# WeijingShi/Point-GNN

Measured on AMD Instinct MI355X. Metric: KITTI-shaped frames/sec (car_auto_T3 inference: graph build + GNN, 20000 pts/frame, mean E1 602k), higher is better.
Workload: dtype f32

## Files before the change

### include/pointgnn_hip.h

```cpp
#ifndef POINTGNN_HIP_H_
#define POINTGNN_HIP_H_

#include <stddef.h>
#include <stdint.h>

#ifdef __cplusplus
extern "C" {
#endif

#define PGNN_E_INVALID (-1)
#define PGNN_E_WORKSPACE (-2)
#define PGNN_E_UNSUPPORTED (-3)
#define PGNN_E_CAPACITY (-4)
#define PGNN_E_COMM (-5)

int pgnn_version(void);
const char *pgnn_last_error(void);
int pgnn_check_device_pointer(const void *device_ptr);

int pgnn_stream_create_cu_mask(int32_t cu_first, int32_t cu_count,
                               int32_t complement, void **stream_out);
int pgnn_stream_destroy(void *stream);

int pgnn_scatter_max_f32(const float *data, int64_t ld_data,
// ... 951 lines not shown
                     const uint8_t *scales, int32_t scale,
                     const uint8_t *colors, int64_t n_colors,
                     const uint8_t *plate_colors, int64_t n_plate_colors,
                     void *workspace, size_t workspace_bytes, void *stream);
int pgnn_render_font(uint8_t *table_host );

size_t pgnn_png_unfilter_workspace_bytes(int64_t width, int64_t height);
int pgnn_png_unfilter(const uint8_t *raw, int64_t width, int64_t height,
                      int32_t color_type, const uint8_t *palette,
                      int32_t palette_entries, int32_t bgr, void *workspace,
                      size_t workspace_bytes, uint8_t *image, void *stream);

size_t pgnn_png_encode_workspace_bytes(int64_t height, int64_t width,
                                       int32_t chunk_bytes);
int pgnn_png_encode(const uint8_t *image, int64_t height, int64_t width,
                    int64_t row_stride_bytes, int32_t chunk_bytes,
                    void *workspace, size_t workspace_bytes, uint8_t *out,
                    int64_t out_capacity, int64_t *out_bytes_dev, void *stream);

int pgnn_set_tunable(const char *key, int value);
int pgnn_kernel_occupancy(const char *kernel, int64_t lds_bytes,
                          int32_t *vgprs, int32_t *scratch_bytes,
                          int32_t *workgroups_per_cu, int64_t *lds_used);
int pgnn_set_debug_buffer(void *device_ptr);

#ifdef __cplusplus
}
#endif
#endif
```

### point-gnn_amd/_lib.py

```python
import ctypes
import os

import torch

from . import _header

_HERE = os.path.dirname(os.path.abspath(__file__))
LIB_PATH = os.environ.get("PGNN_LIB") or os.path.join(_HERE, "libpointgnn_hip.so")

c_i32, c_i64, c_vp = ctypes.c_int32, ctypes.c_int64, ctypes.c_void_p

_S, _C = _header.structs(), _header.constants()

FcLayer = _S["pgnn_fc_layer"]
DynCount = _S["pgnn_dyn_count"]
WgradJob = _S["pgnn_wgrad_job"]
MergeJob = _S["pgnn_merge_job"]
FrameArrays = _S["pgnn_frame_arrays"]
TrainFc = _S["pgnn_train_fc"]
TrainStage = _S["pgnn_train_stage"]
TrainModel = _S["pgnn_train_model"]
TrainBatch = _S["pgnn_train_batch"]


# ... 113 lines not shown
        return ctypes.byref(DynCount(self.dev.data_ptr(), self.hint))


def tag_count(t, count):
    if count is not None:
        t._pgnn_count = count
    return t


def count_of(t):
    return getattr(t, "_pgnn_count", None) if t is not None else None


def kernel_occupancy(kernel, lds_bytes=-1):
    v, sc, wg = c_i32(0), c_i32(0), c_i32(0)
    used = c_i64(0)
    check(load().pgnn_kernel_occupancy(
        kernel.encode(), int(lds_bytes), ctypes.byref(v), ctypes.byref(sc),
        ctypes.byref(wg), ctypes.byref(used)), "pgnn_kernel_occupancy")
    return {"vgprs": v.value, "scratch_bytes": sc.value,
            "workgroups_per_cu": wg.value, "lds_bytes": used.value}


def set_tunable(key, value):
    check(load().pgnn_set_tunable(key.encode(), int(value)), "pgnn_set_tunable")
```

### point-gnn_amd/csrc/gnn.hip

```cpp
#include <atomic>

#include "mlp_engine.h"
#include "edge_ws.h"
#include "edge_ws_split.h"
#include "pool_ws.h"
#include "pool_split.h"
#include "pool_ws_f16.h"

namespace pgnn {
int g_mlp_blocks_per_cu = 4;
int g_edge_msub = 0;
int g_pool_msub = 0;
int g_mlp_pool_pct = 12;
int g_ws_xcds = 8;
int g_ws_prio = 1;
int g_f16_pool = 1;
int g_b16_force = 0;
int g_ws_pool_pct = 0;
int g_ws_chunk = 2;
int g_ws_balance = 1;
int g_ws_reserve = 0;
void *g_mlp_ts = nullptr;
int g_mlp_debug = 0;
}
// ... 2366 lines not shown
      PGNN_REQUIRE(lds_bytes >= 0 && lds_bytes <= 160 * 1024, PGNN_E_INVALID,
                   "kernel_occupancy: no launch of this kernel yet, or more "
                   "LDS than a CU has");
      if (lds_bytes) {
        const int rc = ensure_dynamic_lds(table[i].fn[dyn], (size_t)lds_bytes);
        if (rc) return rc;
      }
      hipFuncAttributes attr;
      PGNN_HIP(hipFuncGetAttributes(&attr, table[i].fn[dyn]));
      int blocks = 0;
      PGNN_HIP(hipOccupancyMaxActiveBlocksPerMultiprocessor(
          &blocks, table[i].fn[dyn], 64 * kRowsWaves, (size_t)lds_bytes));
      *vgprs = attr.numRegs;
      *scratch_bytes = (int32_t)attr.localSizeBytes;
      *workgroups_per_cu = blocks;
      if (lds_used) *lds_used = lds_bytes;
      return 0;
    }
  PGNN_REQUIRE(false, PGNN_E_INVALID, "kernel_occupancy: unknown kernel");
  return 0;
  PGNN_GUARD_END
}

extern "C" int pgnn_point_set_pooling_rows_fwd(
    const float *point_features, int32_t n_feat, const float *point_xyz,
    const int32_t *keypoint_indices, const int32_t *edges, int64_t n_edges,
    int32_t num_keypoints, const pgnn_fc_layer *layers, int32_t n_layers,
    int32_t edges_sorted, float *out, int64_t ld_out, float *const *acts_host,
    int64_t ld_last, void *stream_) {
  PGNN_GUARD_BEGIN
  hipStream_t stream = (hipStream_t)stream_;
  PGNN_REQUIRE(n_edges >= 0 && num_keypoints >= 0 && n_feat >= 0 && n_feat <= 13 &&
                   layers && acts_host,
               PGNN_E_INVALID, "point_set_pooling_rows: bad sizes");
  if (n_layers != 4) return PGNN_E_UNSUPPORTED;
  Plan p;
  int rc = make_plan(layers, n_layers, n_feat + 3, p);
  if (rc) return rc;
  const int out_cols = 16 * p.chain.l[n_layers - 1].nt;
  PGNN_REQUIRE(out && ld_out >= out_cols && ld_last >= out_cols && ld_last % 4 == 0,
               PGNN_E_INVALID, "point_set_pooling_rows: bad output");
  const int cus = ws_cus(stream);
  if (n_edges == 0 || num_keypoints == 0 || !pool_ws_applies(p, n_edges, cus))
    return PGNN_E_UNSUPPORTED;
  PGNN_REQUIRE(point_xyz && keypoint_indices && edges && (n_feat == 0 || point_features),
               PGNN_E_INVALID, "point_set_pooling_rows: null input");
// ... 73 lines not shown
```

### point-gnn_amd/csrc/graph.hip

```cpp
#include <math.h>

#include <mutex>
#include <vector>

#include "kdtree.h"
#include "npy_divmod.h"
#include "sort.h"

namespace pgnn {
namespace {

struct __attribute__((aligned(32))) SortedPoint {
  double x, y, z;
  int32_t idx;
  int32_t pad;
};

__device__ __forceinline__ uint32_t cell_hash(int cx, int cy, int cz,
                                              uint32_t mask) {
  uint32_t h = (uint32_t)cx * 73856093u ^ (uint32_t)cy * 19349663u ^
               (uint32_t)cz * 83492791u;
  h ^= h >> 15;
  return h & mask;
}
// ... 82 lines not shown
                                   int32_t *__restrict__ vcell_sorted,
                                   const int32_t *__restrict__ n_dev) {
  graph_prio();
  if (n_dev) n = *n_dev < n ? *n_dev : n;
  for (int64_t i = (int64_t)blockIdx.x * blockDim.x + threadIdx.x; i < n;
       i += (int64_t)gridDim.x * blockDim.x) {
    const uint32_t k = keys[i];
    if (i == 0 || keys[i - 1] != k) cell_start[k] = (int32_t)i;
    if (i == n - 1 || keys[i + 1] != k) cell_end[k] = (int32_t)(i + 1);
    SortedPoint sp;
    const uint32_t idx = vals[i];
    load_point(pts, idx, sc, sp.x, sp.y, sp.z);
    sp.idx = (int32_t)idx;
    sp.pad = 0;
    sorted[i] = sp;
    if (vcell) {
      vcell_sorted[3 * i] = vcell[3 * (int64_t)idx];
      vcell_sorted[3 * i + 1] = vcell[3 * (int64_t)idx + 1];
      vcell_sorted[3 * i + 2] = vcell[3 * (int64_t)idx + 2];
    }
  }
}

template <bool FILL, typename T>
__global__ __launch_bounds__(1024) void radius_query_kernel(
    const T *__restrict__ centers, int64_t n_centers, Scale3 sc, double r,
    uint32_t mask, const int32_t *__restrict__ cell_start,
    const int32_t *__restrict__ cell_end,
    const SortedPoint *__restrict__ sorted, int32_t *__restrict__ counts,
    const int32_t *__restrict__ offsets, int32_t *__restrict__ edges,
    int64_t capacity, const int32_t *__restrict__ n_centers_dev) {
  graph_prio();
  const int lane = threadIdx.x & 63;
  const int wpb = blockDim.x >> 6;
  const int64_t wave0 = (int64_t)blockIdx.x * wpb + (threadIdx.x >> 6);
  const int64_t n_waves = (int64_t)gridDim.x * wpb;
  const int64_t cap = n_centers;
  if (n_centers_dev)
    n_centers = *n_centers_dev < cap ? *n_centers_dev : cap;
  const double r2 = r * r;
  const double inv_r = 1.0 / r;
  const double rr = r * (1.0 + 1e-9) + 1e-300;
  for (int64_t q = wave0; q < cap; q += n_waves) {
    if (q >= n_centers) {
      if (!FILL && lane == 0) counts[q] = 0;
      continue;
    }
    double cx, cy, cz;
    load_point(centers, q, sc, cx, cy, cz);
    const int x0 = rcell_of(cx - rr, inv_r), x1 = rcell_of(cx + rr, inv_r);
    const int y0 = rcell_of(cy - rr, inv_r), y1 = rcell_of(cy + rr, inv_r);
    const int z0 = rcell_of(cz - rr, inv_r), z1 = rcell_of(cz + rr, inv_r);
    const int nx = x1 - x0 + 1, ny = y1 - y0 + 1, nz = z1 - z0 + 1;
    const int n_cells = nx * ny * nz;
    int my_s = 0, my_cnt = 0, my_ix = 0, my_iy = 0, my_iz = 0;
    if (lane < n_cells) {
      my_ix = x0 + lane % nx;
      my_iy = y0 + (lane / nx) % ny;
      my_iz = z0 + lane / (nx * ny);
      const uint32_t b = cell_hash(my_ix, my_iy, my_iz, mask);
      my_s = cell_start[b];
      my_cnt = cell_end[b] - my_s;
    }
    int incl = my_cnt;
#pragma unroll
    for (int d = 1; d < 64; d <<= 1) {
      const int t = __shfl_up(incl, d);
      if (lane >= d) incl += t;
    }
    const int total_cand = __shfl(incl, 63);
    int64_t out_pos = FILL ? (int64_t)offsets[q] : 0;
    int total = 0;
    for (int j0 = 0; j0 < total_cand; j0 += 128) {
      const bool two = j0 + 64 < total_cand;
      bool valid[2];
      int ix[2], iy[2], iz[2];
      SortedPoint sp[2];
#pragma unroll
      for (int u = 0; u < 2; ++u) {
        if (u == 1 && !two) break;
        valid[u] = j0 + 64 * u + lane < total_cand;
        const int j = valid[u] ? j0 + 64 * u + lane : total_cand - 1;
        int lo = 0, hi = n_cells - 1;
#pragma unroll
        for (int step = 0; step < 6; ++step) {
          const int mid = (lo + hi) >> 1;
          const int v = __shfl(incl, mid);
          if (v > j) hi = mid; else lo = mid + 1;
        }
        const int c = lo < n_cells ? lo : n_cells - 1;
        const int c_incl = __shfl(incl, c), c_cnt = __shfl(my_cnt, c);
        const int c_s = __shfl(my_s, c);
        ix[u] = __shfl(my_ix, c);
// ... 337 lines not shown
  if ((threadIdx.x & 63) == 0) {
    atomicMin(&ordered_min[0], m0);
    atomicMin(&ordered_min[1], m1);
    atomicMin(&ordered_min[2], m2);
  }
}

__global__ void grid_origin_kernel(
    const unsigned long long *__restrict__ ordered_min, double sub_x,
    double sub_y, double sub_z, int mode, double *__restrict__ origin) {
  graph_prio();
  if (threadIdx.x == 0 && blockIdx.x == 0) {
    const double sub[3] = {sub_x, sub_y, sub_z};
    for (int ax = 0; ax < 3; ++ax) {
      const double mn = ordered_to_double(ordered_min[ax]);
      origin[ax] = mn - sub[ax];
      origin[3 + ax] = sub[ax];
      origin[6 + ax] = mn;
    }
    origin[9] = (double)mode;
  }
}

__global__ void voxel_leader_kernel(const SortedPoint *__restrict__ sorted,
                                    const uint32_t *__restrict__ keys, int64_t n,
                                    const int32_t *__restrict__ vc,
                                    const int32_t *__restrict__ cell_start,
                                    const int32_t *__restrict__ cell_end,
                                    int32_t *__restrict__ is_leader,
                                    double *__restrict__ centroid,
                                    int32_t *__restrict__ member_count) {
  graph_prio();
  for (int64_t i = (int64_t)blockIdx.x * blockDim.x + threadIdx.x; i < n;
       i += (int64_t)gridDim.x * blockDim.x) {
    const int vx = vc[3 * i], vy = vc[3 * i + 1], vz = vc[3 * i + 2];
    const uint32_t b = keys[i];
    const int s = cell_start[b], e = cell_end[b];
    bool leader;
    if (vc[3 * s] == vx && vc[3 * s + 1] == vy && vc[3 * s + 2] == vz) {
      leader = (int)i == s;
    } else {
      leader = true;
      for (int j = s; j < (int)i; ++j) {
        if (vc[3 * j] == vx && vc[3 * j + 1] == vy && vc[3 * j + 2] == vz) {
          leader = false;
          break;
        }
      }
    }
    is_leader[i] = leader ? 1 : 0;
    if (!leader) continue;
    double sx = 0.0, sy = 0.0, sz = 0.0;
    int cnt = 0;
    int j = (int)i;
    for (; j + 4 <= e; j += 4) {
      int ax[4], ay[4], az[4];
      SortedPoint o[4];
#pragma unroll
      for (int u = 0; u < 4; ++u) {
        ax[u] = vc[3 * (j + u)];
        ay[u] = vc[3 * (j + u) + 1];
        az[u] = vc[3 * (j + u) + 2];
        o[u] = sorted[j + u];
      }
#pragma unroll
      for (int u = 0; u < 4; ++u) {
        const bool m = ax[u] == vx && ay[u] == vy && az[u] == vz;
        sx = m ? sx + o[u].x : sx;
        sy = m ? sy + o[u].y : sy;
        sz = m ? sz + o[u].z : sz;
        cnt += m ? 1 : 0;
      }
    }
    for (; j < e; ++j) {
      const int ax = vc[3 * j], ay = vc[3 * j + 1], az = vc[3 * j + 2];
      const SortedPoint o = sorted[j];
      const bool m = ax == vx && ay == vy && az == vz;
      sx = m ? sx + o.x : sx;
      sy = m ? sy + o.y : sy;
      sz = m ? sz + o.z : sz;
      cnt += m ? 1 : 0;
    }
    centroid[3 * i] = sx / (double)cnt;
    centroid[3 * i + 1] = sy / (double)cnt;
    centroid[3 * i + 2] = sz / (double)cnt;
    member_count[i] = cnt;
  }
}

__global__ __launch_bounds__(1024) void voxel_nn_kernel(
    const SortedPoint *__restrict__ sorted, int64_t n,
    const double *__restrict__ origin, double voxel, uint32_t mask,
    const int32_t *__restrict__ cell_start, const int32_t *__restrict__ cell_end,
    const int32_t *__restrict__ is_leader, const int32_t *__restrict__ slot,
    const double *__restrict__ centroid, const float *__restrict__ pts,
    KdView kd, int32_t *__restrict__ kp_idx, float *__restrict__ kp_xyz,
    int spw ) {
  graph_prio();
  const int lane = threadIdx.x & 63;
  const int wpb = blockDim.x >> 6;
  const int64_t n_waves = (int64_t)gridDim.x * wpb;
  const double ox = origin[0], oy = origin[1], oz = origin[2];
  for (int64_t base = ((int64_t)blockIdx.x * wpb + (threadIdx.x >> 6)) * spw;
       base < n; base += n_waves * spw) {
    unsigned long long leaders = __ballot(
        lane < spw && base + lane < n && is_leader[base + lane] != 0);
    while (leaders) {
      const int64_t i = base + __builtin_ctzll(leaders);
      leaders &= leaders - 1;
      const double cx = centroid[3 * i], cy = centroid[3 * i + 1],
                   cz = centroid[3 * i + 2];
      const int vx = cell_of(cx, ox, voxel), vy = cell_of(cy, oy, voxel),
                vz = cell_of(cz, oz, voxel);
      int my_s = 0, my_cnt = 0, my_ix = 0, my_iy = 0, my_iz = 0;
      if (lane < 27) {
        my_ix = vx - 1 + lane % 3;
        my_iy = vy - 1 + (lane / 3) % 3;
        my_iz = vz - 1 + lane / 9;
        const uint32_t b = cell_hash(my_ix, my_iy, my_iz, mask);
        my_s = cell_start[b];
        my_cnt = cell_end[b] - my_s;
      }
      int incl = my_cnt;
#pragma unroll
      for (int d = 1; d < 32; d <<= 1) {
        const int t = __shfl_up(incl, d);
        if (lane >= d) incl += t;
      }
      const int total_cand = __shfl(incl, 26);
      double best = 1.0e300;
      int best_idx = 0x7fffffff;
      for (int j0 = 0; j0 < total_cand; j0 += 64) {
        const bool valid = j0 + lane < total_cand;
        const int j = valid ? j0 + lane : total_cand - 1;
        int lo = 0, hi = 26;
#pragma unroll
        for (int step = 0; step < 5; ++step) {
          const int mid = (lo + hi) >> 1;
          const int v = __shfl(incl, mid);
          if (v > j) hi = mid; else lo = mid + 1;
        }
        const int c = lo < 27 ? lo : 26;
        const int c_incl = __shfl(incl, c), c_cnt = __shfl(my_cnt, c);
        const int c_s = __shfl(my_s, c);
        const int ix = __shfl(my_ix, c), iy = __shfl(my_iy, c),
                  iz = __shfl(my_iz, c);
        if (valid) {
          const SortedPoint o = sorted[c_s + (j - (c_incl - c_cnt))];
          if (cell_of(o.x, ox, voxel) == ix && cell_of(o.y, oy, voxel) == iy &&
              cell_of(o.z, oz, voxel) == iz) {
            const double ex = o.x - cx, ey = o.y - cy, ez = o.z - cz;
            const double d2 = (ex * ex + ey * ey) + ez * ez;
// ... 1247 lines not shown
extern "C" int pgnn_voxel_keypoints_random(
    const float *points, int64_t n_points, double voxel_size,
    const double *jitter3_host, uint64_t seed, void *workspace,
    size_t workspace_bytes, int32_t *keypoint_indices, float *keypoint_xyz,
    int32_t *num_keypoints, void *stream) {
  PGNN_GUARD_BEGIN
  return keypoints_impl(points, n_points, voxel_size, false, jitter3_host, seed,
                        workspace, workspace_bytes, keypoint_indices,
                        keypoint_xyz, num_keypoints, (hipStream_t)stream);
  PGNN_GUARD_END
}

extern "C" int pgnn_voxel_keypoints_random_f64(
    const double *points, int64_t n_points, double voxel_size,
    const double *jitter3_host, uint64_t seed, void *workspace,
    size_t workspace_bytes, int32_t *keypoint_indices, double *keypoint_xyz,
    int32_t *num_keypoints, void *stream) {
  PGNN_GUARD_BEGIN
  return keypoints_impl(points, n_points, voxel_size, false, jitter3_host, seed,
                        workspace, workspace_bytes, keypoint_indices,
                        keypoint_xyz, num_keypoints, (hipStream_t)stream);
  PGNN_GUARD_END
}
```

### point-gnn_amd/csrc/kdtree.hip

```cpp
#include "kdtree.h"
#include "pgnn_common.h"

namespace pgnn {
namespace {

struct __attribute__((aligned(16))) Rec {
  float c[3];
  int32_t idx;
};
typedef float kd_v4 __attribute__((ext_vector_type(4)));

#ifndef PGNN_KD_NT
#define PGNN_KD_NT 1024
#endif
#ifndef PGNN_KD_LDS_CAP
#define PGNN_KD_LDS_CAP 5120
#endif
#ifndef PGNN_KD_BATCH
#define PGNN_KD_BATCH 2048
#endif
constexpr int KD_NT = PGNN_KD_NT;
constexpr int KD_NW = KD_NT / 64;
constexpr int KD_LDS_CAP = PGNN_KD_LDS_CAP;
constexpr int KD_BATCH = PGNN_KD_BATCH;
// ... 619 lines not shown
        reinterpret_cast<const void *>(kd_subtree_kernel),
        hipFuncAttributeMaxDynamicSharedMemorySize, (int)dyn));
    attr_set = true;
  }
  hipLaunchKernelGGL(kd_init_kernel, dim3(graph_grid((n + 255) / 256)), dim3(256),
                     graph_lds_pad(), stream, pts, (int)n, rec, kd.status);
  int level0 = 0;
  while (level0 < kd.n_levels - 1 &&
         ((n + ((int64_t)1 << level0) - 1) >> level0) > KD_TOP_LEN) {
    hipLaunchKernelGGL(kd_top_kernel, dim3(graph_grid(1 << level0)), dim3(KD_NT), dyn,
                       stream, rec, (int)n, level0, kd.n_nodes, kd.bounds,
                       kd.status);
    ++level0;
  }
  PGNN_REQUIRE(((n + ((int64_t)1 << level0) - 1) >> level0) <= KD_LDS_CAP,
               PGNN_E_INVALID, "kdtree: leaf larger than the LDS capacity");
  hipLaunchKernelGGL(kd_subtree_kernel, dim3(graph_grid(1 << level0)), dim3(KD_NT), dyn,
                     stream, rec, (int)n, level0, kd.n_levels, kd.n_nodes,
                     kd.bounds, kd.idx, kd.pos, kd.status);
  PGNN_HIP(hipGetLastError());
  return 0;
}

}

using namespace pgnn;

extern "C" int pgnn_kdtree_shape(int64_t n_points, int32_t *n_levels,
                                 int32_t *n_nodes) {
  PGNN_GUARD_BEGIN
  PGNN_REQUIRE(n_points >= 0 && n_levels && n_nodes, PGNN_E_INVALID,
               "kdtree_shape: bad argument");
  int lv, nodes;
  kd_shape(n_points, &lv, &nodes);
  *n_levels = lv;
  *n_nodes = nodes;
  return 0;
  PGNN_GUARD_END
}

extern "C" size_t pgnn_kdtree_workspace_bytes(int64_t n_points) {
  if (n_points < 0) return 0;
  return kd_workspace_bytes(n_points);
}

extern "C" int pgnn_kdtree_replica(const float *points, int64_t n_points,
// ... 26 lines not shown
```

### point-gnn_amd/csrc/pgnn_common.h

```cpp
#pragma once
#include <hip/hip_runtime.h>
#include <stdint.h>
#include <stdio.h>

#include <exception>
#include <string>

#include "pointgnn_hip.h"

namespace pgnn {

std::string &last_error();

inline int fail(int code, const char *msg) {
  last_error() = msg;
  return code;
}

#define PGNN_HIP(expr)                                                        \
  do {                                                                        \
    hipError_t e_ = (expr);                                                   \
    if (e_ != hipSuccess) {                                                   \
      char buf_[256];                                                         \
      snprintf(buf_, sizeof buf_, "%s failed: %s (%s:%d)", #expr,             \
// ... 46 lines not shown
                           __ATOMIC_RELAXED, __HIP_MEMORY_SCOPE_AGENT);
  }
}

#ifndef PGNN_GRAPH_PRIO
#define PGNN_GRAPH_PRIO 0
#endif
__device__ __forceinline__ void graph_prio() {
#if PGNN_GRAPH_PRIO > 0
  __builtin_amdgcn_s_setprio(PGNN_GRAPH_PRIO);
#endif
}

extern int g_graph_lds_pad;
inline size_t graph_lds_pad() { return (size_t)g_graph_lds_pad; }
extern int g_graph_max_wgs;
inline unsigned graph_grid(int64_t natural) {
  if (natural < 1) natural = 1;
  if (g_graph_max_wgs > 0 && natural > g_graph_max_wgs) natural = g_graph_max_wgs;
  return (unsigned)natural;
}
inline unsigned graph_wide_block() { return g_graph_max_wgs > 0 ? 1024u : 256u; }

int device_cu_count();
int stream_cu_count(hipStream_t stream);
int ensure_dynamic_lds(const void *kernel, size_t bytes);
size_t device_max_lds();
int arm_sched(int32_t *sched, hipStream_t stream);

int scatter_sum_strided(const float *data, int64_t ld_data,
                        const int32_t *seg_ids, int64_t seg_stride,
                        int64_t n_rows, int32_t n_cols, int32_t num_segments,
                        float *out, int64_t ld_out, int32_t mean,
                        int32_t *counts_ws, int32_t ids_sorted,
                        hipStream_t stream);
int segment_counts(const int32_t *seg_ids, int64_t seg_stride, int64_t n_rows,
                   const int32_t *n_dev, int32_t num_segments, int32_t *counts,
                   hipStream_t stream);
int segment_mean_finish(float *out, int64_t ld_out, int32_t n_cols,
                        int32_t num_segments, const int32_t *counts,
                        const int32_t *ns_dev, hipStream_t stream);
int mlp_rows_gated(const float *x, int64_t ld_x, int32_t nx, int64_t n_rows,
                   const pgnn_fc_layer *layer, const float *gate, int64_t ld_gate,
                   float *y, int64_t ld_y, hipStream_t stream);
struct RowsTap {
  float *mid;
// ... 9 lines not shown
```

### point-gnn_amd/csrc/sort.hip

```cpp
#include "sort.h"

namespace pgnn {
namespace {

constexpr int kRadix = 256;
constexpr int kSortThreads = 256;
constexpr int kSortItems = kSortTile / kSortThreads;

__device__ __forceinline__ int wave_inclusive_scan(int v, int lane) {
#pragma unroll
  for (int d = 1; d < 64; d <<= 1) {
    int t = __shfl_up(v, d);
    if (lane >= d) v += t;
  }
  return v;
}

__device__ __forceinline__ int block_exclusive_scan(int v, int *total,
                                                    int *lds ) {
  const int lane = threadIdx.x & 63, w = threadIdx.x >> 6;
  const int nw = blockDim.x >> 6;
  int inc = wave_inclusive_scan(v, lane);
  if (lane == 63) lds[w] = inc;
  __syncthreads();
  if (w == 0) {
    int s = (lane < nw) ? lds[lane] : 0;
    int si = wave_inclusive_scan(s, lane);
    if (lane < nw) lds[lane] = si - s;
    if (lane == nw - 1) lds[16] = si;
  }
  __syncthreads();
  int res = inc - v + lds[w];
  *total = lds[16];
  __syncthreads();
  return res;
}

__global__ __launch_bounds__(1024) void scan_single_block_kernel(
    int32_t *data, int64_t n, int32_t *total_out) {
  graph_prio();
  __shared__ int lds[17];
  int carry = 0;
  for (int64_t base = 0; base < n; base += 1024) {
    int64_t i = base + threadIdx.x;
    int v = (i < n) ? data[i] : 0;
    int tot;
    int ex = block_exclusive_scan(v, &tot, lds);
    if (i < n) data[i] = ex + carry;
    carry += tot;
  }
  if (total_out && threadIdx.x == 0) *total_out = carry;
}

constexpr int kScanTile = 4096;

__global__ __launch_bounds__(1024) void scan_tile_sums_kernel(
    const int32_t *in, int64_t n, int32_t *tile_sums, int num_tiles) {
  graph_prio();
  __shared__ int lds[17];
  for (int tile = blockIdx.x; tile < num_tiles; tile += gridDim.x) {
    int64_t base = (int64_t)tile * kScanTile + threadIdx.x * 4;
    int s = 0;
#pragma unroll
    for (int k = 0; k < 4; ++k)
      if (base + k < n) s += in[base + k];
    int tot;
    block_exclusive_scan(s, &tot, lds);
    if (threadIdx.x == 0) tile_sums[tile] = tot;
  }
}

__global__ __launch_bounds__(1024) void scan_tiles_kernel(
    const int32_t *in, int32_t *out, int64_t n, const int32_t *tile_offsets,
    int num_tiles) {
  graph_prio();
  __shared__ int lds[17];
  for (int tile = blockIdx.x; tile < num_tiles; tile += gridDim.x) {
    int64_t base = (int64_t)tile * kScanTile + threadIdx.x * 4;
    int v[4];
    int s = 0;
#pragma unroll
    for (int k = 0; k < 4; ++k) {
      v[k] = (base + k < n) ? in[base + k] : 0;
      s += v[k];
    }
    int tot;
    int ex = block_exclusive_scan(s, &tot, lds) + tile_offsets[tile];
#pragma unroll
    for (int k = 0; k < 4; ++k) {
      if (base + k < n) out[base + k] = ex;
      ex += v[k];
    }
    if (base <= n - 1 && n - 1 < base + 4) out[n] = ex;
  }
}

__global__ __launch_bounds__(kSortThreads) void radix_hist_kernel(
    const uint32_t *__restrict__ keys, int64_t n, int shift,
    int32_t *__restrict__ block_hist , int num_tiles,
    const int32_t *__restrict__ n_dev ) {
  graph_prio();
  if (n_dev) n = *n_dev < n ? *n_dev : n;
  __shared__ int hist[kRadix];
  for (int tile = blockIdx.x; tile < num_tiles; tile += gridDim.x) {
    hist[threadIdx.x] = 0;
    __syncthreads();
    const int64_t base = (int64_t)tile * kSortTile;
#pragma unroll
    for (int i = 0; i < kSortItems; ++i) {
      int64_t idx = base + i * kSortThreads + threadIdx.x;
      if (idx < n) atomicAdd(&hist[(keys[idx] >> shift) & (kRadix - 1)], 1);
    }
    __syncthreads();
    block_hist[(int64_t)threadIdx.x * num_tiles + tile] = hist[threadIdx.x];
  }
}
// ... 52 lines not shown

size_t radix_sort_scratch_bytes(int64_t n) {
  int64_t tiles = (n + kSortTile - 1) / kSortTile;
  if (tiles < 1) tiles = 1;
  return align_up((size_t)tiles * kRadix * sizeof(int32_t), 256) + 256;
}

int radix_sort_pairs(uint32_t *keys_a, uint32_t *vals_a, uint32_t *keys_b,
                     uint32_t *vals_b, int64_t n, int nbits, void *scratch,
                     size_t scratch_bytes, uint32_t **keys_out,
                     uint32_t **vals_out, hipStream_t stream,
                     const int32_t *n_dev) {
  *keys_out = keys_a;
  *vals_out = vals_a;
  if (n <= 0) return 0;
  PGNN_REQUIRE(scratch_bytes >= radix_sort_scratch_bytes(n), PGNN_E_WORKSPACE,
               "radix sort: scratch too small");
  const int num_tiles = (int)((n + kSortTile - 1) / kSortTile);
  int32_t *hist = (int32_t *)scratch;
  uint32_t *kin = keys_a, *vin = vals_a, *kout = keys_b, *vout = vals_b;
  for (int shift = 0; shift < nbits; shift += 8) {
    hipLaunchKernelGGL(radix_hist_kernel, dim3(graph_grid(num_tiles)), dim3(kSortThreads), graph_lds_pad(),
                       stream, kin, n, shift, hist, num_tiles, n_dev);
    hipLaunchKernelGGL(scan_single_block_kernel, dim3(1), dim3(1024), graph_lds_pad(), stream,
                       hist, (int64_t)kRadix * num_tiles, (int32_t *)nullptr);
    hipLaunchKernelGGL(radix_scatter_kernel, dim3(graph_grid(num_tiles)),
                       dim3(kSortThreads), graph_lds_pad(), stream, kin, vin, kout, vout, n,
                       shift, hist, num_tiles, n_dev);
    uint32_t *tk = kin, *tv = vin;
    kin = kout;
    vin = vout;
    kout = tk;
    vout = tv;
  }
  PGNN_HIP(hipGetLastError());
  *keys_out = kin;
  *vals_out = vin;
  return 0;
}

size_t scan_scratch_bytes(int64_t n) {
  int64_t tiles = (n + kScanTile - 1) / kScanTile;
  if (tiles < 1) tiles = 1;
  return align_up((size_t)(tiles + 1) * sizeof(int32_t), 256);
}

int exclusive_scan_i32(const int32_t *in, int32_t *out, int64_t n,
                       void *scratch, size_t scratch_bytes,
                       hipStream_t stream) {
  if (n <= 0) {
    PGNN_HIP(hipMemsetAsync(out, 0, sizeof(int32_t), stream));
    return 0;
  }
  PGNN_REQUIRE(scratch_bytes >= scan_scratch_bytes(n), PGNN_E_WORKSPACE,
               "scan: scratch too small");
  const int num_tiles = (int)((n + kScanTile - 1) / kScanTile);
  int32_t *tile_sums = (int32_t *)scratch;
  hipLaunchKernelGGL(scan_tile_sums_kernel, dim3(graph_grid(num_tiles)), dim3(1024), graph_lds_pad(),
                     stream, in, n, tile_sums, num_tiles);
  hipLaunchKernelGGL(scan_single_block_kernel, dim3(1), dim3(1024), graph_lds_pad(), stream,
                     tile_sums, (int64_t)num_tiles, (int32_t *)nullptr);
  hipLaunchKernelGGL(scan_tiles_kernel, dim3(graph_grid(num_tiles)), dim3(1024), graph_lds_pad(), stream,
                     in, out, n, tile_sums, num_tiles);
  PGNN_HIP(hipGetLastError());
  return 0;
}

int exclusive_scan_inplace_i32(int32_t *data, int64_t n, hipStream_t stream) {
  if (n <= 0) return 0;
  hipLaunchKernelGGL(scan_single_block_kernel, dim3(1), dim3(1024), graph_lds_pad(), stream,
                     data, n, (int32_t *)nullptr);
  PGNN_HIP(hipGetLastError());
  return 0;
}

}
```

### point-gnn_amd/csrc/ws_launch.h

```cpp
#pragma once
#include "ws_partition.h"

namespace {
using namespace pgnn;

inline int ws_cus(int cus) {
  return (g_ws_reserve > 0 && cus - g_ws_reserve >= 64) ? cus - g_ws_reserve : cus;
}
inline int ws_cus(hipStream_t stream) { return ws_cus(stream_cu_count(stream)); }

inline int ws_slices(int cus) { return ws_slice_count(cus, g_ws_xcds); }
inline bool ws_feasible(int nt, int ntmax, int cus) {
  return pgnn::ws_feasible(nt, ntmax, cus, ws_slices(cus));
}

inline int ws_partition_rc(int why) {
  PGNN_REQUIRE(why != kWsTooFewCus, PGNN_E_UNSUPPORTED,
               "edge_ws: too few CUs for the column groups");
  PGNN_REQUIRE(why == kWsOk, PGNN_E_UNSUPPORTED,
               "edge_ws: column tiles do not group");
  return 0;
}

template <int KQ, int NTMAX>
int plan_edge_ws(EdgeWsArgs &a, const LayerDev &L, const EdgeArgs &ea,
                 int64_t n_edges, const SegArgs &sa, int cus, int32_t *sched,
                 float *rows_out, int64_t ld_rows, float *h1_out,
// ... 17 lines not shown
  a.ldo = sa.ldo;
  a.num_segments = sa.num_segments;
  a.sorted = sa.sorted;
  a.prio = g_ws_prio;
  a.ts = (long long *)g_mlp_ts;
  a.sched = (g_ws_pool_pct > 0 && a.xcds <= kWsMaxSlices) ? sched : nullptr;
  a.pool_pct = g_ws_pool_pct;
  a.chunk = g_ws_chunk;
  if (g_ws_balance >= 2) {
    double cost[kWsMaxGroups];
    for (int g = 0; g < a.groups; ++g)
      cost[g] = 128.0 * KQ * (a.tile0[g + 1] - a.tile0[g]) + 1900.0;
    ws_balance(a, cus, cost, a.sched != nullptr);
  }
  return 0;
}

template <int KQ, int NTMAX, bool ROWS, class POL = WsMax, bool SCALED = false,
          bool K300 = false>
int run_edge_ws(const EdgeWsArgs &a, int cus, hipStream_t stream) {
  static_assert(!POL::kSum || !ROWS, "the sum kernels read no ready rows");
  static_assert(!SCALED || (!POL::kSum && !ROWS), "scaled: the plain max kernel only");
  PGNN_HIP((hipError_t)arm_sched(a.sched, stream));
  const size_t lds = (size_t)KQ * NTMAX * 1024 + 16 * NTMAX * sizeof(float);
  auto kern = edge_ws_kernel<KQ, NTMAX, false, ROWS, POL, SCALED, K300>;
  if constexpr (!ROWS && !POL::kSum && !SCALED) {
    if (a.rows_out) kern = edge_ws_kernel<KQ, NTMAX, true>;
  }
  return launch_lds(kern, dim3((unsigned)(cus / a.xcds * a.xcds)),
                    dim3(64 * kWsWaves), lds, stream, a);
}

template <int KQ, int NTMAX, class POL = WsMax>
int launch_edge_ws(const LayerDev &L, const EdgeArgs &ea, int64_t n_edges,
                   const SegArgs &sa, int cus, int32_t *sched,
                   hipStream_t stream, float *rows_out = nullptr,
                   int64_t ld_rows = 0, float *h1_out = nullptr,
                   const int32_t *n_dev = nullptr) {
  EdgeWsArgs a;
  const int rc = plan_edge_ws<KQ, NTMAX>(a, L, ea, n_edges, sa, cus, sched,
                                         rows_out, ld_rows, h1_out, n_dev);
  return rc ? rc : run_edge_ws<KQ, NTMAX, false, POL>(a, cus, stream);
}

template <int KQ, int NTMAX, bool K300 = false>
int launch_edge_ws_scaled(const LayerDev &L, const EdgeArgs &ea, int64_t n_edges,
                          const SegArgs &sa, int cus, int32_t *sched,
// ... 73 lines not shown
  a.pool_pct = g_ws_pool_pct;
  a.chunk = 1;
  PGNN_HIP((hipError_t)arm_sched(a.sched, stream));
  return 0;
}

template <class POL = WsMax>
int launch_pool_ws(const Plan &p, const PoolArgs &pa, int64_t n_edges,
                   const SegArgs &sa, int cus, int32_t *sched,
                   hipStream_t stream, float *const *acts = nullptr,
                   int64_t ld4 = 0, const int32_t *n_dev = nullptr) {
  PoolWsArgs a = pool_ws_args(p, pa, n_edges, n_dev, sa.num_segments);
  if (acts) {
    a.a1_out = acts[0];
    a.a2_out = acts[1];
    a.a3_out = acts[2];
    a.a4_out = acts[3];
    a.ld4 = ld4;
  }
  a.prio = g_ws_prio;
  a.ts = (long long *)g_mlp_ts;
  const int rc = pool_ws_out(a, sa, sched, stream);
  if (rc) return rc;
  const size_t lds = (size_t)8 * 19 * 1024 + 16 * 19 * sizeof(float);
  auto kern = pool_ws_kernel<false, POL>;
  if constexpr (!POL::kSum) {
    if (acts) kern = pool_ws_kernel<true>;
  }
  return launch_lds(kern, dim3((unsigned)cus), dim3(64 * kWsWaves), lds, stream,
                    a);
}

constexpr int kPoolSplitHidden = 256;
bool pool_split_applies(const Plan &p, int64_t n_edges, int cus) {
  if (g_mlp_debug & (8192 | 1024)) return false;
  const ChainDev &c = p.chain;
  if (c.n != 5 || c.l[0].kq != 1 || c.l[0].nt != 2 || c.l[1].nt != 4 ||
      c.l[2].nt != 8 || c.l[3].kq != 8 || c.l[3].nt != 16 || c.l[4].kq != 16 ||
      c.l[4].nt != 32)
    return false;
  if (cus < 64 || cus % 8 != 0) return false;
  if (!ws_feasible(c.l[4].nt, 8, cus)) return false;
  if ((size_t)16 * 8 * 1024 + 16 * 16 * sizeof(float) > device_max_lds())
    return false;
  if (g_mlp_debug & 16384) return true;
  return n_edges >= (int64_t)16 * 2 * kWsWaves * cus;
}
// ... 126 lines not shown
```

Measured before the change: 331.7.

## Add kernel footprint API, vectorize scans, mark wave-uniform values in graph kernels

Adds a kernel-footprint query API and exported scan/radix-sort entry points. Scan kernels drop from 1024 to 256 threads and use int4 vectorized loads and stores with more items per thread. The radius-query and voxel-nn kernels wrap per-wave values in readfirstlane so the compiler can keep them in scalar registers and free vector registers. The voxel leader loop unroll falls from 4 to 2 and loads only the xyz fields, which lowers register pressure but reduces memory-level parallelism.

```diff
diff --git a/include/pointgnn_hip.h b/include/pointgnn_hip.h
--- a/include/pointgnn_hip.h
+++ b/include/pointgnn_hip.h
@@ -997,6 +997,19 @@
 int pgnn_kernel_occupancy(const char *kernel, int64_t lds_bytes,
                           int32_t *vgprs, int32_t *scratch_bytes,
                           int32_t *workgroups_per_cu, int64_t *lds_used);
+int pgnn_kernel_footprint(const char *kernel, int32_t *vgprs,
+                          int32_t *scratch_bytes, int32_t *static_lds_bytes,
+                          int32_t *block_threads, int64_t *dynamic_lds_bytes);
+const char *pgnn_kernel_footprint_name(int32_t index);
+size_t pgnn_scan_workspace_bytes(int64_t n);
+int pgnn_exclusive_scan_i32(const int32_t *in, int32_t *out, int64_t n,
+                            void *workspace, size_t workspace_bytes,
+                            void *stream);
+int pgnn_exclusive_scan_inplace_i32(int32_t *data, int64_t n, void *stream);
+size_t pgnn_radix_sort_workspace_bytes(int64_t n);
+int pgnn_radix_sort_pairs(uint32_t *keys, uint32_t *vals, uint32_t *keys_tmp,
+                          uint32_t *vals_tmp, int64_t n, int32_t nbits,
+                          void *workspace, size_t workspace_bytes, void *stream);
 int pgnn_set_debug_buffer(void *device_ptr);
 
 #ifdef __cplusplus
diff --git a/point-gnn_amd/_lib.py b/point-gnn_amd/_lib.py
--- a/point-gnn_amd/_lib.py
+++ b/point-gnn_amd/_lib.py
@@ -159,5 +159,26 @@
             "workgroups_per_cu": wg.value, "lds_bytes": used.value}
 
 
+def kernel_footprint_names():
+    lib, names, i = load(), [], 0
+    while True:
+        s = lib.pgnn_kernel_footprint_name(i)
+        if s is None:
+            return names
+        names.append(s.decode())
+        i += 1
+
+
+def kernel_footprint(kernel):
+    v, sc, lds, blk = c_i32(0), c_i32(0), c_i32(0), c_i32(0)
+    dyn = c_i64(0)
+    check(load().pgnn_kernel_footprint(
+        kernel.encode(), ctypes.byref(v), ctypes.byref(sc), ctypes.byref(lds),
+        ctypes.byref(blk), ctypes.byref(dyn)), "pgnn_kernel_footprint")
+    return {"vgprs": v.value, "scratch_bytes": sc.value,
+            "static_lds_bytes": lds.value, "block_threads": blk.value,
+            "dynamic_lds_bytes": dyn.value}
+
+
 def set_tunable(key, value):
     check(load().pgnn_set_tunable(key.encode(), int(value)), "pgnn_set_tunable")
diff --git a/point-gnn_amd/csrc/gnn.hip b/point-gnn_amd/csrc/gnn.hip
--- a/point-gnn_amd/csrc/gnn.hip
+++ b/point-gnn_amd/csrc/gnn.hip
@@ -2412,6 +2412,63 @@
   PGNN_GUARD_END
 }
 
+extern "C" const char *pgnn_kernel_footprint_name(int32_t index) {
+  if (index < 0) return nullptr;
+  const KernelRow *(*const tables[3])(int *) = {graph_kernel_rows, sort_kernel_rows,
+                                                kd_kernel_rows};
+  for (auto table : tables) {
+    int n = 0;
+    const KernelRow *rows = table(&n);
+    if (index < n) return rows[index].name;
+    index -= n;
+  }
+  return index == 0 ? "edge_ws_k300" : index == 1 ? "pool_ws" : nullptr;
+}
+
+extern "C" int pgnn_kernel_footprint(const char *kernel, int32_t *vgprs,
+                                     int32_t *scratch_bytes,
+                                     int32_t *static_lds_bytes,
+                                     int32_t *block_threads,
+                                     int64_t *dynamic_lds_bytes) {
+  PGNN_GUARD_BEGIN
+  PGNN_REQUIRE(kernel && vgprs && scratch_bytes && static_lds_bytes &&
+                   block_threads && dynamic_lds_bytes,
+               PGNN_E_INVALID, "kernel_footprint: null argument");
+  const std::string name(kernel);
+  const void *fn = nullptr;
+  if (name == "edge_ws_k300") {
+    fn = reinterpret_cast<const void *>(
+        edge_ws_kernel<19, 7, false, false, WsMax, true, true>);
+    *block_threads = 64 * kWsWaves;
+    *dynamic_lds_bytes = (int64_t)edge_ws_lds_bytes(19, 7);
+  } else if (name == "pool_ws") {
+    fn = reinterpret_cast<const void *>(pool_ws_kernel<false, WsMax>);
+    *block_threads = 64 * kWsWaves;
+    *dynamic_lds_bytes = (int64_t)kPoolWsLdsBytes;
+  } else {
+    const KernelRow *(*const tables[3])(int *) = {
+        graph_kernel_rows, sort_kernel_rows, kd_kernel_rows};
+    for (auto table : tables) {
+      int n = 0;
+      const KernelRow *rows = table(&n);
+      for (int i = 0; i < n && !fn; ++i)
+        if (name == rows[i].name) {
+          fn = rows[i].fn;
+          *block_threads = rows[i].block ? rows[i].block : (int)graph_wide_block();
+        }
+    }
+    *dynamic_lds_bytes = (int64_t)graph_lds_pad();
+  }
+  PGNN_REQUIRE(fn, PGNN_E_INVALID, "kernel_footprint: unknown kernel");
+  hipFuncAttributes attr;
+  PGNN_HIP(hipFuncGetAttributes(&attr, fn));
+  *vgprs = attr.numRegs;
+  *scratch_bytes = (int32_t)attr.localSizeBytes;
+  *static_lds_bytes = (int32_t)attr.sharedSizeBytes;
+  return 0;
+  PGNN_GUARD_END
+}
+
 extern "C" int pgnn_point_set_pooling_rows_fwd(
     const float *point_features, int32_t n_feat, const float *point_xyz,
     const int32_t *keypoint_indices, const int32_t *edges, int64_t n_edges,
diff --git a/point-gnn_amd/csrc/graph.hip b/point-gnn_amd/csrc/graph.hip
--- a/point-gnn_amd/csrc/graph.hip
+++ b/point-gnn_amd/csrc/graph.hip
@@ -128,6 +128,14 @@
   }
 }
 
+__device__ __forceinline__ int wave_uniform(int v) {
+  return __builtin_amdgcn_readfirstlane(v);
+}
+__device__ __forceinline__ double wave_uniform(double v) {
+  return __hiloint2double(wave_uniform(__double2hiint(v)),
+                          wave_uniform(__double2loint(v)));
+}
+
 template <bool FILL, typename T>
 __global__ __launch_bounds__(1024) void radius_query_kernel(
     const T *__restrict__ centers, int64_t n_centers, Scale3 sc, double r,
@@ -139,14 +147,15 @@
   graph_prio();
   const int lane = threadIdx.x & 63;
   const int wpb = blockDim.x >> 6;
-  const int64_t wave0 = (int64_t)blockIdx.x * wpb + (threadIdx.x >> 6);
+  const int64_t wave0 =
+      (int64_t)blockIdx.x * wpb + wave_uniform((int)(threadIdx.x >> 6));
   const int64_t n_waves = (int64_t)gridDim.x * wpb;
   const int64_t cap = n_centers;
   if (n_centers_dev)
     n_centers = *n_centers_dev < cap ? *n_centers_dev : cap;
-  const double r2 = r * r;
-  const double inv_r = 1.0 / r;
-  const double rr = r * (1.0 + 1e-9) + 1e-300;
+  const double r2 = wave_uniform(r * r);
+  const double inv_r = wave_uniform(1.0 / r);
+  const double rr = wave_uniform(r * (1.0 + 1e-9) + 1e-300);
   for (int64_t q = wave0; q < cap; q += n_waves) {
     if (q >= n_centers) {
       if (!FILL && lane == 0) counts[q] = 0;
@@ -154,9 +163,15 @@
     }
     double cx, cy, cz;
     load_point(centers, q, sc, cx, cy, cz);
-    const int x0 = rcell_of(cx - rr, inv_r), x1 = rcell_of(cx + rr, inv_r);
-    const int y0 = rcell_of(cy - rr, inv_r), y1 = rcell_of(cy + rr, inv_r);
-    const int z0 = rcell_of(cz - rr, inv_r), z1 = rcell_of(cz + rr, inv_r);
+    cx = wave_uniform(cx);
+    cy = wave_uniform(cy);
+    cz = wave_uniform(cz);
+    const int x0 = wave_uniform(rcell_of(cx - rr, inv_r)),
+              x1 = wave_uniform(rcell_of(cx + rr, inv_r));
+    const int y0 = wave_uniform(rcell_of(cy - rr, inv_r)),
+              y1 = wave_uniform(rcell_of(cy + rr, inv_r));
+    const int z0 = wave_uniform(rcell_of(cz - rr, inv_r)),
+              z1 = wave_uniform(rcell_of(cz + rr, inv_r));
     const int nx = x1 - x0 + 1, ny = y1 - y0 + 1, nz = z1 - z0 + 1;
     const int n_cells = nx * ny * nz;
     int my_s = 0, my_cnt = 0, my_ix = 0, my_iy = 0, my_iz = 0;
@@ -174,7 +189,7 @@
       const int t = __shfl_up(incl, d);
       if (lane >= d) incl += t;
     }
-    const int total_cand = __shfl(incl, 63);
+    const int total_cand = wave_uniform(__shfl(incl, 63));
     int64_t out_pos = FILL ? (int64_t)offsets[q] : 0;
     int total = 0;
     for (int j0 = 0; j0 < total_cand; j0 += 128) {
@@ -558,6 +573,7 @@
   }
 }
 
+constexpr int kLeaderSlots = 2;
 __global__ void voxel_leader_kernel(const SortedPoint *__restrict__ sorted,
                                     const uint32_t *__restrict__ keys, int64_t n,
                                     const int32_t *__restrict__ vc,
@@ -589,22 +605,24 @@
     double sx = 0.0, sy = 0.0, sz = 0.0;
     int cnt = 0;
     int j = (int)i;
-    for (; j + 4 <= e; j += 4) {
-      int ax[4], ay[4], az[4];
-      SortedPoint o[4];
-#pragma unroll
-      for (int u = 0; u < 4; ++u) {
+    for (; j + kLeaderSlots <= e; j += kLeaderSlots) {
+      int ax[kLeaderSlots], ay[kLeaderSlots], az[kLeaderSlots];
+      double ox[kLeaderSlots], oy[kLeaderSlots], oz[kLeaderSlots];
+#pragma unroll
+      for (int u = 0; u < kLeaderSlots; ++u) {
         ax[u] = vc[3 * (j + u)];
         ay[u] = vc[3 * (j + u) + 1];
         az[u] = vc[3 * (j + u) + 2];
-        o[u] = sorted[j + u];
-      }
-#pragma unroll
-      for (int u = 0; u < 4; ++u) {
+        ox[u] = sorted[j + u].x;
+        oy[u] = sorted[j + u].y;
+        oz[u] = sorted[j + u].z;
+      }
+#pragma unroll
+      for (int u = 0; u < kLeaderSlots; ++u) {
         const bool m = ax[u] == vx && ay[u] == vy && az[u] == vz;
-        sx = m ? sx + o[u].x : sx;
-        sy = m ? sy + o[u].y : sy;
-        sz = m ? sz + o[u].z : sz;
+        sx = m ? sx + ox[u] : sx;
+        sy = m ? sy + oy[u] : sy;
+        sz = m ? sz + oz[u] : sz;
         cnt += m ? 1 : 0;
       }
     }
@@ -637,17 +655,20 @@
   const int wpb = blockDim.x >> 6;
   const int64_t n_waves = (int64_t)gridDim.x * wpb;
   const double ox = origin[0], oy = origin[1], oz = origin[2];
-  for (int64_t base = ((int64_t)blockIdx.x * wpb + (threadIdx.x >> 6)) * spw;
+  for (int64_t base = ((int64_t)blockIdx.x * wpb +
+                       wave_uniform((int)(threadIdx.x >> 6))) * spw;
        base < n; base += n_waves * spw) {
     unsigned long long leaders = __ballot(
         lane < spw && base + lane < n && is_leader[base + lane] != 0);
     while (leaders) {
       const int64_t i = base + __builtin_ctzll(leaders);
       leaders &= leaders - 1;
-      const double cx = centroid[3 * i], cy = centroid[3 * i + 1],
-                   cz = centroid[3 * i + 2];
-      const int vx = cell_of(cx, ox, voxel), vy = cell_of(cy, oy, voxel),
-                vz = cell_of(cz, oz, voxel);
+      const double cx = wave_uniform(centroid[3 * i]),
+                   cy = wave_uniform(centroid[3 * i + 1]),
+                   cz = wave_uniform(centroid[3 * i + 2]);
+      const int vx = wave_uniform(cell_of(cx, ox, voxel)),
+                vy = wave_uniform(cell_of(cy, oy, voxel)),
+                vz = wave_uniform(cell_of(cz, oz, voxel));
       int my_s = 0, my_cnt = 0, my_ix = 0, my_iy = 0, my_iz = 0;
       if (lane < 27) {
         my_ix = vx - 1 + lane % 3;
@@ -663,7 +684,7 @@
         const int t = __shfl_up(incl, d);
         if (lane >= d) incl += t;
       }
-      const int total_cand = __shfl(incl, 26);
+      const int total_cand = wave_uniform(__shfl(incl, 26));
       double best = 1.0e300;
       int best_idx = 0x7fffffff;
       for (int j0 = 0; j0 < total_cand; j0 += 64) {
@@ -1957,3 +1978,32 @@
                         keypoint_xyz, num_keypoints, (hipStream_t)stream);
   PGNN_GUARD_END
 }
+
+namespace pgnn {
+const KernelRow *graph_kernel_rows(int *n) {
+#define PGNN_ROW(name, kernel, block) \
+  {name, reinterpret_cast<const void *>(kernel), block}
+  static const KernelRow rows[] = {
+      PGNN_ROW("cell_keys_kernel<float>", cell_keys_kernel<float>, 256),
+      PGNN_ROW("cell_bounds_kernel<float>", cell_bounds_kernel<float>, 256),
+      PGNN_ROW("radius_query_kernel<false, float>",
+               (radius_query_kernel<false, float>), 0),
+      PGNN_ROW("radius_query_kernel<true, float>",
+               (radius_query_kernel<true, float>), 0),
+      PGNN_ROW("radius_query_kernel<false, double>",
+               (radius_query_kernel<false, double>), 0),
+      PGNN_ROW("radius_query_kernel<true, double>",
+               (radius_query_kernel<true, double>), 0),
+      PGNN_ROW("edge_total_kernel", edge_total_kernel, 64),
+      PGNN_ROW("min_bound_kernel<float>", min_bound_kernel<float>, 256),
+      PGNN_ROW("grid_origin_kernel", grid_origin_kernel, 64),
+      PGNN_ROW("voxel_leader_kernel", voxel_leader_kernel, 256),
+      PGNN_ROW("copy_total_kernel", copy_total_kernel, 64),
+      PGNN_ROW("voxel_nn_kernel", voxel_nn_kernel, 0),
+      PGNN_ROW("graph_fill32_kernel", graph_fill32_kernel, 1024),
+  };
+#undef PGNN_ROW
+  *n = (int)(sizeof(rows) / sizeof(rows[0]));
+  return rows;
+}
+}
diff --git a/point-gnn_amd/csrc/kdtree.hip b/point-gnn_amd/csrc/kdtree.hip
--- a/point-gnn_amd/csrc/kdtree.hip
+++ b/point-gnn_amd/csrc/kdtree.hip
@@ -665,6 +665,17 @@
   return 0;
 }
 
+const KernelRow *kd_kernel_rows(int *n) {
+  static const KernelRow rows[] = {
+      {"kd_init_kernel", reinterpret_cast<const void *>(kd_init_kernel), 256},
+      {"kd_top_kernel", reinterpret_cast<const void *>(kd_top_kernel), KD_NT},
+      {"kd_subtree_kernel", reinterpret_cast<const void *>(kd_subtree_kernel),
+       KD_NT},
+  };
+  *n = (int)(sizeof(rows) / sizeof(rows[0]));
+  return rows;
+}
+
 }
 
 using namespace pgnn;
diff --git a/point-gnn_amd/csrc/pgnn_common.h b/point-gnn_amd/csrc/pgnn_common.h
--- a/point-gnn_amd/csrc/pgnn_common.h
+++ b/point-gnn_amd/csrc/pgnn_common.h
@@ -92,6 +92,15 @@
 }
 inline unsigned graph_wide_block() { return g_graph_max_wgs > 0 ? 1024u : 256u; }
 
+struct KernelRow {
+  const char *name;
+  const void *fn;
+  int block;
+};
+const KernelRow *graph_kernel_rows(int *n);
+const KernelRow *sort_kernel_rows(int *n);
+const KernelRow *kd_kernel_rows(int *n);
+
 int device_cu_count();
 int stream_cu_count(hipStream_t stream);
 int ensure_dynamic_lds(const void *kernel, size_t bytes);
diff --git a/point-gnn_amd/csrc/sort.hip b/point-gnn_amd/csrc/sort.hip
--- a/point-gnn_amd/csrc/sort.hip
+++ b/point-gnn_amd/csrc/sort.hip
@@ -6,6 +6,8 @@
 constexpr int kRadix = 256;
 constexpr int kSortThreads = 256;
 constexpr int kSortItems = kSortTile / kSortThreads;
+
+constexpr int kScanThreads = 256;
 
 __device__ __forceinline__ int wave_inclusive_scan(int v, int lane) {
 #pragma unroll
@@ -36,62 +38,122 @@
   return res;
 }
 
-__global__ __launch_bounds__(1024) void scan_single_block_kernel(
+template <int ITEMS>
+__device__ __forceinline__ void load_run(const int32_t *p, int64_t base,
+                                         int64_t n, bool aligned, int (&v)[ITEMS]) {
+  if (aligned && base + ITEMS <= n) {
+#pragma unroll
+    for (int k = 0; k < ITEMS; k += 4) {
+      const int4 q = *reinterpret_cast<const int4 *>(p + base + k);
+      v[k] = q.x;
+      v[k + 1] = q.y;
+      v[k + 2] = q.z;
+      v[k + 3] = q.w;
+    }
+  } else {
+#pragma unroll
+    for (int k = 0; k < ITEMS; ++k) v[k] = (base + k < n) ? p[base + k] : 0;
+  }
+}
+
+__device__ __forceinline__ bool aligned16(const void *p) {
+  return ((uintptr_t)p & 15) == 0;
+}
+
+constexpr int kScanSingleItems = 4;
+constexpr int kScanSingleTile = kScanThreads * kScanSingleItems;
+
+__global__ __launch_bounds__(kScanThreads) void scan_single_block_kernel(
     int32_t *data, int64_t n, int32_t *total_out) {
   graph_prio();
   __shared__ int lds[17];
+  const bool al = aligned16(data);
   int carry = 0;
-  for (int64_t base = 0; base < n; base += 1024) {
-    int64_t i = base + threadIdx.x;
-    int v = (i < n) ? data[i] : 0;
+  for (int64_t base = 0; base < n; base += kScanSingleTile) {
+    const int64_t i = base + (int64_t)threadIdx.x * kScanSingleItems;
+    int v[kScanSingleItems];
+    load_run(data, i, n, al, v);
+    int s = 0;
+#pragma unroll
+    for (int k = 0; k < kScanSingleItems; ++k) s += v[k];
     int tot;
-    int ex = block_exclusive_scan(v, &tot, lds);
-    if (i < n) data[i] = ex + carry;
+    int ex = block_exclusive_scan(s, &tot, lds) + carry;
+    if (al && i + kScanSingleItems <= n) {
+      int4 q;
+      q.x = ex;
+      q.y = q.x + v[0];
+      q.z = q.y + v[1];
+      q.w = q.z + v[2];
+      *reinterpret_cast<int4 *>(data + i) = q;
+    } else {
+#pragma unroll
+      for (int k = 0; k < kScanSingleItems; ++k) {
+        if (i + k < n) data[i + k] = ex;
+        ex += v[k];
+      }
+    }
     carry += tot;
   }
   if (total_out && threadIdx.x == 0) *total_out = carry;
 }
 
 constexpr int kScanTile = 4096;
-
-__global__ __launch_bounds__(1024) void scan_tile_sums_kernel(
+constexpr int kScanItems = kScanTile / kScanThreads;
+
+__global__ __launch_bounds__(kScanThreads) void scan_tile_sums_kernel(
     const int32_t *in, int64_t n, int32_t *tile_sums, int num_tiles) {
   graph_prio();
   __shared__ int lds[17];
+  const bool al = aligned16(in);
   for (int tile = blockIdx.x; tile < num_tiles; tile += gridDim.x) {
-    int64_t base = (int64_t)tile * kScanTile + threadIdx.x * 4;
+    const int64_t base =
+        (int64_t)tile * kScanTile + (int64_t)threadIdx.x * kScanItems;
+    int v[kScanItems];
+    load_run(in, base, n, al, v);
     int s = 0;
 #pragma unroll
-    for (int k = 0; k < 4; ++k)
-      if (base + k < n) s += in[base + k];
+    for (int k = 0; k < kScanItems; ++k) s += v[k];
     int tot;
     block_exclusive_scan(s, &tot, lds);
     if (threadIdx.x == 0) tile_sums[tile] = tot;
   }
 }
 
-__global__ __launch_bounds__(1024) void scan_tiles_kernel(
+__global__ __launch_bounds__(kScanThreads) void scan_tiles_kernel(
     const int32_t *in, int32_t *out, int64_t n, const int32_t *tile_offsets,
     int num_tiles) {
   graph_prio();
   __shared__ int lds[17];
+  const bool al_in = aligned16(in), al_out = aligned16(out);
   for (int tile = blockIdx.x; tile < num_tiles; tile += gridDim.x) {
-    int64_t base = (int64_t)tile * kScanTile + threadIdx.x * 4;
-    int v[4];
+    const int64_t base =
+        (int64_t)tile * kScanTile + (int64_t)threadIdx.x * kScanItems;
+    int v[kScanItems];
+    load_run(in, base, n, al_in, v);
     int s = 0;
 #pragma unroll
-    for (int k = 0; k < 4; ++k) {
-      v[k] = (base + k < n) ? in[base + k] : 0;
-      s += v[k];
-    }
+    for (int k = 0; k < kScanItems; ++k) s += v[k];
     int tot;
     int ex = block_exclusive_scan(s, &tot, lds) + tile_offsets[tile];
-#pragma unroll
-    for (int k = 0; k < 4; ++k) {
-      if (base + k < n) out[base + k] = ex;
-      ex += v[k];
-    }
-    if (base <= n - 1 && n - 1 < base + 4) out[n] = ex;
+    if (al_out && base + kScanItems <= n) {
+#pragma unroll
+      for (int k = 0; k < kScanItems; k += 4) {
+        int4 q;
+        q.x = ex;
+        q.y = q.x + v[k];
+        q.z = q.y + v[k + 1];
+        q.w = q.z + v[k + 2];
+        ex = q.w + v[k + 3];
+        *reinterpret_cast<int4 *>(out + base + k) = q;
+      }
+    } else {
+#pragma unroll
+      for (int k = 0; k < kScanItems; ++k) {
+        if (base + k < n) out[base + k] = ex;
+        ex += v[k];
+      }
+    }
+    if (base <= n - 1 && n - 1 < base + kScanItems) out[n] = ex;
   }
 }
 
@@ -190,7 +252,7 @@
   for (int shift = 0; shift < nbits; shift += 8) {
     hipLaunchKernelGGL(radix_hist_kernel, dim3(graph_grid(num_tiles)), dim3(kSortThreads), graph_lds_pad(),
                        stream, kin, n, shift, hist, num_tiles, n_dev);
-    hipLaunchKernelGGL(scan_single_block_kernel, dim3(1), dim3(1024), graph_lds_pad(), stream,
+    hipLaunchKernelGGL(scan_single_block_kernel, dim3(1), dim3(kScanThreads), graph_lds_pad(), stream,
                        hist, (int64_t)kRadix * num_tiles, (int32_t *)nullptr);
     hipLaunchKernelGGL(radix_scatter_kernel, dim3(graph_grid(num_tiles)),
                        dim3(kSortThreads), graph_lds_pad(), stream, kin, vin, kout, vout, n,
@@ -224,22 +286,96 @@
                "scan: scratch too small");
   const int num_tiles = (int)((n + kScanTile - 1) / kScanTile);
   int32_t *tile_sums = (int32_t *)scratch;
-  hipLaunchKernelGGL(scan_tile_sums_kernel, dim3(graph_grid(num_tiles)), dim3(1024), graph_lds_pad(),
+  hipLaunchKernelGGL(scan_tile_sums_kernel, dim3(graph_grid(num_tiles)), dim3(kScanThreads), graph_lds_pad(),
                      stream, in, n, tile_sums, num_tiles);
-  hipLaunchKernelGGL(scan_single_block_kernel, dim3(1), dim3(1024), graph_lds_pad(), stream,
+  hipLaunchKernelGGL(scan_single_block_kernel, dim3(1), dim3(kScanThreads), graph_lds_pad(), stream,
                      tile_sums, (int64_t)num_tiles, (int32_t *)nullptr);
-  hipLaunchKernelGGL(scan_tiles_kernel, dim3(graph_grid(num_tiles)), dim3(1024), graph_lds_pad(), stream,
+  hipLaunchKernelGGL(scan_tiles_kernel, dim3(graph_grid(num_tiles)), dim3(kScanThreads), graph_lds_pad(), stream,
                      in, out, n, tile_sums, num_tiles);
   PGNN_HIP(hipGetLastError());
   return 0;
 }
 
+const KernelRow *sort_kernel_rows(int *n) {
+  static const KernelRow rows[] = {
+      {"scan_single_block_kernel",
+       reinterpret_cast<const void *>(scan_single_block_kernel), kScanThreads},
+      {"scan_tile_sums_kernel",
+       reinterpret_cast<const void *>(scan_tile_sums_kernel), kScanThreads},
+      {"scan_tiles_kernel", reinterpret_cast<const void *>(scan_tiles_kernel),
+       kScanThreads},
+      {"radix_hist_kernel", reinterpret_cast<const void *>(radix_hist_kernel),
+       kSortThreads},
+      {"radix_scatter_kernel",
+       reinterpret_cast<const void *>(radix_scatter_kernel), kSortThreads},
+  };
+  *n = (int)(sizeof(rows) / sizeof(rows[0]));
+  return rows;
+}
+
 int exclusive_scan_inplace_i32(int32_t *data, int64_t n, hipStream_t stream) {
   if (n <= 0) return 0;
-  hipLaunchKernelGGL(scan_single_block_kernel, dim3(1), dim3(1024), graph_lds_pad(), stream,
+  hipLaunchKernelGGL(scan_single_block_kernel, dim3(1), dim3(kScanThreads), graph_lds_pad(), stream,
                      data, n, (int32_t *)nullptr);
   PGNN_HIP(hipGetLastError());
   return 0;
 }
 
 }
+
+extern "C" size_t pgnn_scan_workspace_bytes(int64_t n) {
+  return pgnn::scan_scratch_bytes(n);
+}
+
+extern "C" int pgnn_exclusive_scan_i32(const int32_t *in, int32_t *out,
+                                       int64_t n, void *workspace,
+                                       size_t workspace_bytes, void *stream) {
+  PGNN_GUARD_BEGIN
+  PGNN_REQUIRE(n >= 0 && n < ((int64_t)1 << 31) && out && (n == 0 || in) &&
+                   in != out,
+               PGNN_E_INVALID, "exclusive_scan: bad arguments");
+  PGNN_REQUIRE(n == 0 || workspace, PGNN_E_WORKSPACE,
+               "exclusive_scan: null workspace");
+  return pgnn::exclusive_scan_i32(in, out, n, workspace, workspace_bytes,
+                                  (hipStream_t)stream);
+  PGNN_GUARD_END
+}
+
+extern "C" int pgnn_exclusive_scan_inplace_i32(int32_t *data, int64_t n,
+                                               void *stream) {
+  PGNN_GUARD_BEGIN
+  PGNN_REQUIRE(n >= 0 && (n == 0 || data), PGNN_E_INVALID,
+               "exclusive_scan_inplace: bad arguments");
+  return pgnn::exclusive_scan_inplace_i32(data, n, (hipStream_t)stream);
+  PGNN_GUARD_END
+}
+
+extern "C" size_t pgnn_radix_sort_workspace_bytes(int64_t n) {
+  return pgnn::radix_sort_scratch_bytes(n);
+}
+
+extern "C" int pgnn_radix_sort_pairs(uint32_t *keys, uint32_t *vals,
+                                     uint32_t *keys_tmp, uint32_t *vals_tmp,
+                                     int64_t n, int32_t nbits, void *workspace,
+                                     size_t workspace_bytes, void *stream_) {
+  PGNN_GUARD_BEGIN
+  hipStream_t stream = (hipStream_t)stream_;
+  PGNN_REQUIRE(n >= 0 && n < ((int64_t)1 << 31) && nbits >= 1 && nbits <= 32,
+               PGNN_E_INVALID, "radix_sort_pairs: bad sizes");
+  if (n == 0) return 0;
+  PGNN_REQUIRE(keys && vals && keys_tmp && vals_tmp && workspace, PGNN_E_INVALID,
+               "radix_sort_pairs: null argument");
+  uint32_t *ko = nullptr, *vo = nullptr;
+  const int rc = pgnn::radix_sort_pairs(keys, vals, keys_tmp, vals_tmp, n, nbits,
+                                        workspace, workspace_bytes, &ko, &vo,
+                                        stream);
+  if (rc) return rc;
+  if (ko != keys) {
+    PGNN_HIP(hipMemcpyAsync(keys, ko, (size_t)n * sizeof(uint32_t),
+                            hipMemcpyDeviceToDevice, stream));
+    PGNN_HIP(hipMemcpyAsync(vals, vo, (size_t)n * sizeof(uint32_t),
+                            hipMemcpyDeviceToDevice, stream));
+  }
+  return 0;
+  PGNN_GUARD_END
+}
diff --git a/point-gnn_amd/csrc/ws_launch.h b/point-gnn_amd/csrc/ws_launch.h
--- a/point-gnn_amd/csrc/ws_launch.h
+++ b/point-gnn_amd/csrc/ws_launch.h
@@ -3,6 +3,11 @@
 
 namespace {
 using namespace pgnn;
+
+constexpr size_t edge_ws_lds_bytes(int kq, int ntmax) {
+  return (size_t)kq * ntmax * 1024 + 16 * ntmax * sizeof(float);
+}
+constexpr size_t kPoolWsLdsBytes = (size_t)8 * 19 * 1024 + 16 * 19 * sizeof(float);
 
 inline int ws_cus(int cus) {
   return (g_ws_reserve > 0 && cus - g_ws_reserve >= 64) ? cus - g_ws_reserve : cus;
@@ -66,7 +71,7 @@
   static_assert(!POL::kSum || !ROWS, "the sum kernels read no ready rows");
   static_assert(!SCALED || (!POL::kSum && !ROWS), "scaled: the plain max kernel only");
   PGNN_HIP((hipError_t)arm_sched(a.sched, stream));
-  const size_t lds = (size_t)KQ * NTMAX * 1024 + 16 * NTMAX * sizeof(float);
+  const size_t lds = edge_ws_lds_bytes(KQ, NTMAX);
   auto kern = edge_ws_kernel<KQ, NTMAX, false, ROWS, POL, SCALED, K300>;
   if constexpr (!ROWS && !POL::kSum && !SCALED) {
     if (a.rows_out) kern = edge_ws_kernel<KQ, NTMAX, true>;
@@ -186,7 +191,7 @@
   a.ts = (long long *)g_mlp_ts;
   const int rc = pool_ws_out(a, sa, sched, stream);
   if (rc) return rc;
-  const size_t lds = (size_t)8 * 19 * 1024 + 16 * 19 * sizeof(float);
+  const size_t lds = kPoolWsLdsBytes;
   auto kern = pool_ws_kernel<false, POL>;
   if constexpr (!POL::kSum) {
     if (acts) kern = pool_ws_kernel<true>;
```

Result: no change. 334.4 (median of 6 runs) (+0.8%).
